# zyc-123/InstanceDiff

Hardware: AMD Instinct MI355X
Metric: denoising steps/sec (256x256 bs16) (higher is better)
Workload: dtype f32; 1 GPU; 256x256 1-ch synthetic, 1000-step reverse chain, batch 16 per GPU, 2 UNet fwd + reverse update per step; global_batch=16, parallelism=replicas x1 (no collective)

## Files before the change

### include/idiff.h

```cpp
#ifndef IDIFF_H
#define IDIFF_H

#include <stdint.h>

#ifdef __cplusplus
extern "C" {
#endif

#define IDIFF_OK 0
#define IDIFF_E_BADARG (-1)
#define IDIFF_E_UNSUPPORTED (-2)
#define IDIFF_E_HIP (-3)

typedef void* idiff_stream_t;

const char* idiff_last_error(void);
int idiff_version(void);
int64_t idiff_launch_count(void);
int idiff_device_info(int* num_cu, int* wave_size, char* arch_name, int arch_name_len);

#define IDIFF_CONV_NORMAL 0
#define IDIFF_CONV_UPSAMPLE2 1
#define IDIFF_CONV_UNSHUFFLE2 2

// ... 79 lines not shown
    const float* res;
    int64_t ldr;
    const float* gscale;
    float* out;
    int64_t ldo;
    const float* ln_g;
    const float* ln_b;
    float ln_eps;
    int32_t R, K, N, act_in, act_out;
} idiff_linear_group;
int idiff_linear_t_grouped_fwd(const idiff_linear_group* groups, int ngroups, idiff_stream_t stream);
int idiff_linear_t_ln_fwd(const float* x, int64_t ldx, const float* ln_g, const float* ln_b, float ln_eps, const float* wT,
                          int64_t ldw, const float* bias, const float* res, int64_t ldr, const float* gscale, float* out,
                          int64_t ldo, int R, int K, int N, int act_out, idiff_stream_t stream);
int idiff_linear_t_heads_fwd(const float* x, int64_t ldx, int64_t x_hs, const float* wT, int64_t ldw, int64_t w_hs,
                             const float* bias, int64_t b_hs, float* out, int64_t ldo, int64_t o_hs, int R, int K, int N,
                             int heads, idiff_stream_t stream);
int idiff_smm_memproj_fwd(const float* feat, int64_t feat_bstride, const float* ln1_g, const float* ln1_b,
                          const float* wpk, const float* bias, const float* ln2_g, const float* ln2_b, float* out, int B,
                          int C, int N, float eps, idiff_stream_t stream);
int idiff_smm_memproj_compact_fwd(const float* feat, int64_t feat_bstride, const float* ln1_g, const float* ln1_b,
                                  const float* gram, const float* hvec, float evar, float* out, int B, int C, int N, int Cm,
                                  float eps1, float eps2, idiff_stream_t stream);
int idiff_smm_memproj_compact_train_fwd(const float* feat, int64_t feat_bstride, const float* ln1_g, const float* ln1_b, const float* gram,
                                        const float* hvec, const float* evar_dev, float* out, int B, int C, int N, int Cm, float eps1,
                                        float eps2, idiff_stream_t stream);
int64_t idiff_smm_memproj_compact_bwd_ws_floats(int B, int C, int N);
int idiff_smm_memproj_compact_bwd(const float* feat, int64_t feat_bstride, const float* ln1_g, const float* ln1_b, const float* gram,
                                  const float* hvec, const float* evar_dev, const float* dm, float* dfeat, int64_t dfeat_bstride,
                                  float* dparams, float* ws, int B, int C, int N, int Cm, float eps1, float eps2, idiff_stream_t stream);
#define IDIFF_MEMPROJ_MAX_GROUPS 4
typedef struct idiff_memproj_group {
    const float* feat;
    int64_t feat_bstride;
    const float *ln1_g, *ln1_b, *gram, *hvec;
    float evar;
    float* out;
    int32_t C, N, Cm;
} idiff_memproj_group;
int idiff_smm_memproj_compact_grouped_fwd(const idiff_memproj_group* groups, int ngroups, int B, float eps1, float eps2,
                                          idiff_stream_t stream);
int idiff_layernorm_rows_fwd(const float* x, int64_t ldx, const float* gamma, const float* beta, float* out,
                             int64_t ldo, int R, int C, float eps, float* mean_rstd, idiff_stream_t stream);
int idiff_time_embed_fwd(const float* t, const float* freqs, int B, int dim, float* out, idiff_stream_t stream);
int idiff_time_mlp_fwd(const float* t, const float* freqs, const float* w0, const float* b0, const float* w2, const float* b2, float* out,
                       int B, int dim, int hid, int nout, idiff_stream_t stream);

int idiff_chan_layernorm_fwd(const float* x, int64_t x_bstride, const float* gamma, const float* beta, float* out,
                             int64_t out_bstride, int B, int C, int HW, float eps, float* mean_rstd,
                             idiff_stream_t stream);

int idiff_attn_self_fwd(const float* qkv, float* out, float* lse, int B, int C, int N, int heads, float scale,
                        idiff_stream_t stream);
int idiff_attn_self_bf16_fwd(const float* qkv, float* out, int B, int C, int N, int heads, float scale, idiff_stream_t stream);
int idiff_attn_self_f16_fwd(const float* qkv, float* out, int B, int C, int N, int heads, float scale, idiff_stream_t stream);
int idiff_attn_ctx_fwd(const float* q, const float* k, const float* v, float* out, int B, int C, int N, int M,
                       int heads, float scale, idiff_stream_t stream);
int idiff_attn_tokens_fwd(const float* q, const float* k, const float* v, float* out, int B, int Nq, int M, int C,
                          int heads, float scale, int64_t ldq, int64_t ldkv, idiff_stream_t stream);
int idiff_attn_tokens_bwd(const float* q, const float* k, const float* v, const float* d_o, float* dq, float* dk, float* dv, int B, int Nq,
                          int M, int C, int heads, float scale, int64_t ldq, int64_t ldkv, int64_t ldo, int64_t lddq, int64_t lddkv,
                          idiff_stream_t stream);
int idiff_attn_tokens_grouped_fwd(const float* const* q, const float* const* k, const float* const* v, float* const* out, int ngroups,
                                  int B, int Nq, int M, int C, int heads, float scale, int64_t ldq, int64_t ldkv, idiff_stream_t stream);
int idiff_attn_tokens_f16_fwd(const float* q, const float* k, const float* v, float* out, int B, int Nq, int M, int C, int heads, float scale,
                              int64_t ldq, int64_t ldkv, idiff_stream_t stream);
int64_t idiff_smm_xattn_kv_f16_ws_floats(int B, int N);
int idiff_smm_xattn_kv_f16_fwd(const float* q, const float* k, const float* v, float* out, float* ws, int B, int Nq, int heads, int C, int N,
                               float scale, idiff_stream_t stream);
int64_t idiff_smm_xattn_ws_floats(int B, int Nq, int heads, int Cm, int N);
int idiff_smm_xattn_fwd(const float* qf, const float* mem, float* o, float* ws, int B, int Nq, int heads, int Cm,
                        int N, float scale, idiff_stream_t stream);
#define IDIFF_XATTN_MAX_GROUPS 8
typedef struct idiff_xattn_group {
    const float* qf;
    const float* mem;
    float* o;
    float* ws;
    int32_t Cm, N;
} idiff_xattn_group;
int idiff_smm_xattn_grouped_fwd(const idiff_xattn_group* groups, int ngroups, int B, int Nq, int heads, float scale,
                                idiff_stream_t stream);
int idiff_smm_xattn_lse_fwd(const float* qf, const float* mem, float* o, float* lse, float* ws, int B, int rows, int N, float scale,
                            idiff_stream_t stream);
int idiff_smm_xattn_bwd(const float* qf, const float* mem, const float* o, const float* lse, const float* d_o, float* dqf, float* dmem,
                        int accumulate, float* ws, int B, int rows, int N, float scale, idiff_stream_t stream);
int idiff_smm_xattn_cm_lse_fwd(const float* qf, const float* mem, float* o, float* lse, float* ws, int B, int rows, int Cm, int N,
                               float scale, idiff_stream_t stream);
int idiff_smm_xattn_cm_bwd(const float* qf, const float* mem, const float* o, const float* lse, const float* d_o, float* dqf, float* dmem,
                           int accumulate, float* ws, int B, int rows, int Cm, int N, float scale, idiff_stream_t stream);
int idiff_scoremap_fwd(const float* feat, int64_t feat_bstride, const float* tv, float* out, const int32_t* idx,
                       float* sel, int B, int C, int HW, int K, idiff_stream_t stream);
#define IDIFF_SCOREMAP_MAX_GROUPS 4
typedef struct idiff_scoremap_group {
    const float* feat;
    int64_t feat_bstride;
    const float* tv;
    float* out;
    float* sel;
    int32_t C, HW;
} idiff_scoremap_group;
int idiff_scoremap_grouped_fwd(const idiff_scoremap_group* groups, int ngroups, const int32_t* idx, int B, int K, idiff_stream_t stream);
int idiff_conv3x3_select_fwd(const float* x, int64_t x_bstride, const float* w, const float* bias, const int32_t* idx, float* out,
                             int B, int C, int K, int H, int W, idiff_stream_t stream);
int64_t idiff_conv3x3_select_bwd_ws_floats(int B, int C, int H, int W);
int idiff_conv3x3_select_bwd(const float* x, int64_t x_bstride, const float* w, const int32_t* idx, const float* dpred, float* dx,
// ... 112 lines not shown
```

### instancediff_amd/_lib.py

```python
import ctypes as C
import os
import re

_HERE = os.path.dirname(os.path.abspath(__file__))
LIB_PATH = os.environ.get("IDIFF_LIB") or os.path.join(_HERE, "libidiff_hip.so")
HEADER_PATH = os.path.join(os.path.dirname(_HERE), "include", "idiff.h")

c_f32p = C.c_void_p
c_stream = C.c_void_p


class ConvDesc(C.Structure):
    _fields_ = [
        ("src0", C.c_void_p), ("src1", C.c_void_p),
        ("src0_bstride", C.c_int64), ("src1_bstride", C.c_int64),
        ("C0", C.c_int32), ("C1", C.c_int32),
        ("B", C.c_int32), ("Hin", C.c_int32), ("Win", C.c_int32),
        ("mode", C.c_int32), ("ks", C.c_int32), ("Cout", C.c_int32),
        ("wpk", C.c_void_p), ("bias", C.c_void_p),
        ("pro_a", C.c_void_p), ("pro_b", C.c_void_p),
        ("out", C.c_void_p), ("out_bstride", C.c_int64),
        ("res", C.c_void_p), ("res_bstride", C.c_int64),
        ("vec", C.c_void_p),
        ("aux", C.c_void_p), ("aux_bstride", C.c_int64), ("aux_a", C.c_void_p), ("aux_b", C.c_void_p),
# ... 15 lines not shown

class XattnGroup(C.Structure):
    _fields_ = [("qf", C.c_void_p), ("mem", C.c_void_p), ("o", C.c_void_p), ("ws", C.c_void_p), ("Cm", C.c_int32), ("N", C.c_int32)]


class MemprojGroup(C.Structure):
    _fields_ = [("feat", C.c_void_p), ("feat_bstride", C.c_int64), ("ln1_g", C.c_void_p), ("ln1_b", C.c_void_p), ("gram", C.c_void_p),
                ("hvec", C.c_void_p), ("evar", C.c_float), ("out", C.c_void_p), ("C", C.c_int32), ("N", C.c_int32), ("Cm", C.c_int32)]


class ScoremapGroup(C.Structure):
    _fields_ = [("feat", C.c_void_p), ("feat_bstride", C.c_int64), ("tv", C.c_void_p), ("out", C.c_void_p), ("sel", C.c_void_p),
                ("C", C.c_int32), ("HW", C.c_int32)]


LINEAR_MAX_GROUPS = 16
XATTN_MAX_GROUPS, MEMPROJ_MAX_GROUPS, SCOREMAP_MAX_GROUPS = 8, 4, 4
P, I, I64, F, U64 = C.c_void_p, C.c_int, C.c_int64, C.c_float, C.c_uint64

SIGNATURES = {
    "idiff_last_error": (C.c_char_p, []),
    "idiff_version": (I, []),
    "idiff_launch_count": (I64, []),
    "idiff_device_info": (I, [C.POINTER(I), C.POINTER(I), C.c_char_p, I]),
    "idiff_conv2d_num_tiles": (I, [I, I]),
    "idiff_conv2d_fwd": (I, [C.POINTER(ConvDesc), c_stream]),
    "idiff_conv2d_last_algo": (I, []),
    "idiff_conv2d_plan": (I, [C.POINTER(ConvDesc)]),
    "idiff_pack_conv_weight": (I, [P, P, I, I, I, c_stream]),
    "idiff_pack_conv_weight_T": (I, [P, P, I, I, I, c_stream]),
    "idiff_pack_conv_weight_wino": (I, [P, P, I, I, I, c_stream]),
    "idiff_pack_conv_weight_wino4": (I, [P, P, I, I, I, c_stream]),
    "idiff_conv1x1_x3_image_bytes": (C.c_longlong, [I, I]),
    "idiff_pack_conv1x1_x3": (I, [P, P, I, I, c_stream]),
    "idiff_gn_finalize": (I, [P, I, I, I, I, I, P, P, P, I64, F, P, P, P, c_stream]),
    "idiff_affine_silu_add": (I, [P, I64, P, P, P, I64, P, P, I64, I, I, I, c_stream]),
    "idiff_linear_fwd": (I, [P, I64, P, I64, P, P, I64, P, P, I64, I, I, I, I, I, c_stream]),
    "idiff_linear_t_fwd": (I, [P, I64, P, I64, P, P, I64, P, P, I64, I, I, I, I, I, c_stream]),
    "idiff_linear_t_ln_fwd": (I, [P, I64, P, P, F, P, I64, P, P, I64, P, P, I64, I, I, I, I, c_stream]),
    "idiff_linear_t_grouped_fwd": (I, [C.POINTER(LinearGroup), I, c_stream]),
    "idiff_attn_tokens_grouped_fwd": (I, [C.POINTER(P), C.POINTER(P), C.POINTER(P), C.POINTER(P), I, I, I, I, I, I, F, I64, I64, c_stream]),
    "idiff_linear_t_heads_fwd": (I, [P, I64, I64, P, I64, I64, P, I64, P, I64, I64, I, I, I, I, c_stream]),
    "idiff_smm_memproj_fwd": (I, [P, I64, P, P, P, P, P, P, P, I, I, I, F, c_stream]),
    "idiff_smm_memproj_compact_fwd": (I, [P, I64, P, P, P, P, F, P, I, I, I, I, F, F, c_stream]),
    "idiff_smm_memproj_compact_train_fwd": (I, [P, I64, P, P, P, P, P, P, I, I, I, I, F, F, c_stream]),
    "idiff_smm_memproj_compact_bwd_ws_floats": (I64, [I, I, I]),
    "idiff_smm_memproj_compact_bwd": (I, [P, I64, P, P, P, P, P, P, P, I64, P, P, I, I, I, I, F, F, c_stream]),
    "idiff_smm_memproj_compact_grouped_fwd": (I, [C.POINTER(MemprojGroup), I, I, F, F, c_stream]),
    "idiff_layernorm_rows_fwd": (I, [P, I64, P, P, P, I64, I, I, F, P, c_stream]),
    "idiff_time_embed_fwd": (I, [P, P, I, I, P, c_stream]),
    "idiff_time_mlp_fwd": (I, [P, P, P, P, P, P, P, I, I, I, I, c_stream]),
    "idiff_chan_layernorm_fwd": (I, [P, I64, P, P, P, I64, I, I, I, F, P, c_stream]),
    "idiff_attn_self_fwd": (I, [P, P, P, I, I, I, I, F, c_stream]),
    "idiff_attn_self_bf16_fwd": (I, [P, P, I, I, I, I, F, c_stream]),
    "idiff_attn_self_f16_fwd": (I, [P, P, I, I, I, I, F, c_stream]),
    "idiff_attn_ctx_fwd": (I, [P, P, P, P, I, I, I, I, I, F, c_stream]),
    "idiff_attn_tokens_fwd": (I, [P, P, P, P, I, I, I, I, I, F, I64, I64, c_stream]),
    "idiff_attn_tokens_bwd": (I, [P, P, P, P, P, P, P, I, I, I, I, I, F, I64, I64, I64, I64, I64, c_stream]),
    "idiff_smm_xattn_ws_floats": (I64, [I, I, I, I, I]),
    "idiff_attn_tokens_f16_fwd": (I, [P, P, P, P, I, I, I, I, I, F, I64, I64, c_stream]),
    "idiff_smm_xattn_kv_f16_ws_floats": (I64, [I, I]),
    "idiff_smm_xattn_kv_f16_fwd": (I, [P, P, P, P, P, I, I, I, I, I, F, c_stream]),
    "idiff_smm_xattn_fwd": (I, [P, P, P, P, I, I, I, I, I, F, c_stream]),
    "idiff_smm_xattn_grouped_fwd": (I, [C.POINTER(XattnGroup), I, I, I, I, F, c_stream]),
    "idiff_smm_xattn_lse_fwd": (I, [P, P, P, P, P, I, I, I, F, c_stream]),
    "idiff_smm_xattn_bwd": (I, [P, P, P, P, P, P, P, I, P, I, I, I, F, c_stream]),
    "idiff_smm_xattn_cm_lse_fwd": (I, [P, P, P, P, P, I, I, I, I, F, c_stream]),
    "idiff_smm_xattn_cm_bwd": (I, [P, P, P, P, P, P, P, I, P, I, I, I, I, F, c_stream]),
    "idiff_scoremap_fwd": (I, [P, I64, P, P, P, P, I, I, I, I, c_stream]),
    "idiff_scoremap_grouped_fwd": (I, [C.POINTER(ScoremapGroup), I, P, I, I, c_stream]),
    "idiff_gather_channel": (I, [P, P, P, I, I, I, c_stream]),
    "idiff_conv3x3_select_fwd": (I, [P, I64, P, P, P, P, I, I, I, I, I, c_stream]),
    "idiff_conv3x3_select_bwd_ws_floats": (I64, [I, I, I, I]),
    "idiff_conv3x3_select_bwd": (I, [P, I64, P, P, P, P, I64, P, P, P, I, I, I, I, I, c_stream]),
    "idiff_irsde_reverse_step": (I, [P, P, P, P, P, I64, F, F, F, F, F, I, U64, U64, c_stream]),
    "idiff_irsde_map": (I, [I, P, P, P, P, F, P, I, I64, P, C.POINTER(C.c_float), U64, U64, c_stream]),
    "idiff_drift_reverse_step": (I, [P, P, P, P, P, P, P, I64, F, F, F, U64, U64, c_stream]),
    "idiff_drift_reverse_step_dev": (I, [P, P, P, P, P, P, I64, P, I, P, U64, U64, U64, c_stream]),
    "idiff_step_state_advance": (I, [P, P, I, I, I, c_stream]),
    "idiff_randn": (I, [P, I64, U64, U64, c_stream]),
    "idiff_dropout": (I, [P, P, I64, F, U64, U64, c_stream]),
    "idiff_philox_raw": (I, [P, I64, U64, U64, c_stream]),
    "idiff_axpby": (I, [P, P, P, I64, F, F, c_stream]),
    "idiff_mix3_per_sample": (I, [P, P, P, P, P, P, P, I, I64, c_stream]),
    "idiff_conv2d_wgrad_ws_floats": (I64, [C.POINTER(ConvDesc)]),
    "idiff_conv2d_wgrad": (I, [C.POINTER(ConvDesc), P, I64, P, I, P, c_stream]),
    "idiff_conv2d_wgrad_last_algo": (I, []),
    "idiff_sumpool2x2": (I, [P, P, I64, I, I, c_stream]),
    "idiff_pixel_shuffle2": (I, [P, P, I, I, I, I, c_stream]),
    "idiff_plane_sum": (I, [P, I64, P, I, I, I, c_stream]),
    "idiff_batch_sum": (I, [P, P, I, I, I, c_stream]),
    "idiff_sum_n": (I, [C.POINTER(P), C.POINTER(I64), I, P, I64, I, I64, c_stream]),
    "idiff_gather_segments": (I, [P, I, I64, P, c_stream]),
    "idiff_gn_silu_bwd_ws_floats": (I64, [I, I, I]),
    "idiff_gn_silu_bwd": (I, [P, I64, P, I64, P, P, P, P, P, P, I64, P, I64, P, P, P, I64, P, I, I, I, I, I, P, P, c_stream]),
    "idiff_act_fwd": (I, [P, P, I64, I, c_stream]),
    "idiff_act_bwd": (I, [P, P, P, I64, I, c_stream]),
    "idiff_colsum": (I, [P, I64, P, I, I, I, c_stream]),
    "idiff_scale_cols": (I, [P, P, P, I, I, c_stream]),
    "idiff_colsum_prod": (I, [P, P, P, I, I, c_stream]),
    "idiff_layernorm_rows_bwd": (I, [P, I64, P, I64, P, P, P, I64, P, P, I, I, I, c_stream]),
    "idiff_chan_layernorm_bwd_ws_floats": (I64, [I, I, I]),
    "idiff_chan_layernorm_bwd": (I, [P, I64, P, I64, P, P, P, I64, P, P, P, I, I, I, I, c_stream]),
    "idiff_chan_normalize_fwd": (I, [P, I64, P, P, I, I, I, c_stream]),
    "idiff_chan_normalize_bwd": (I, [P, P, P, P, I64, I, I, I, c_stream]),
    "idiff_scatter_channel": (I, [P, P, P, I, I, I, c_stream]),
# ... 57 lines not shown
```

### instancediff_amd/csrc/attention.hip

```cpp
#include <math.h>
#include <type_traits>
#include <stdlib.h>

#include "common.h"

namespace {

#define KAPPA(r) (((r) & 3) + 8 * ((r) >> 2))

template <int DH>
__global__ __launch_bounds__(256) void attn_self_kernel(const float* __restrict__ qkv, float* __restrict__ out, float* __restrict__ lse, int C,
                                                        int N, int heads, float scale) {
    constexpr int MB = DH / 32;
    constexpr int KT = DH * 32;
    constexpr int VT = DH * 33;
    constexpr int BUF = KT + VT + 3;
    constexpr int NV4 = DH * 32 / 4 / 256;
    extern __shared__ __attribute__((aligned(16))) float smem[];

    const int tid = threadIdx.x, lane = tid & 63, wave = tid >> 6, half = lane >> 5, l31 = lane & 31;
    const int b = blockIdx.y / heads, h = blockIdx.y % heads;
    const int q0 = (blockIdx.x * 4 + wave) * 32;
    const float* qb = qkv + (long long)b * 3 * C * N + (long long)(h * DH) * N;
    const float* kb = qb + (long long)C * N;
    const float* vb = qb + (long long)2 * C * N;

    float qreg[DH / 2];
    const int qi = q0 + l31;
#pragma unroll
    for (int s = 0; s < DH / 2; ++s) qreg[s] = qi < N ? qb[(long long)(2 * s + half) * N + qi] : 0.f;

    floatx16 O[MB];
#pragma unroll
    for (int m = 0; m < MB; ++m)
#pragma unroll
        for (int r = 0; r < 16; ++r) O[m][r] = 0.f;
    float mrun = -INFINITY, lrun = 0.f;

    const int nkb = (N + 31) / 32;
    floatx4 rk[NV4], rv[NV4];
    auto load_tile = [&](int kbi) {
        const int key0 = kbi * 32;
#pragma unroll
        for (int i = 0; i < NV4; ++i) {
            const int f = tid + i * 256;
            const int d = f >> 3, j4 = (f & 7) * 4;
            floatx4 kz = {0.f, 0.f, 0.f, 0.f}, vz = {0.f, 0.f, 0.f, 0.f};
            if (key0 + j4 + 3 < N) {
                kz = *reinterpret_cast<const floatx4*>(kb + (long long)d * N + key0 + j4);
                vz = *reinterpret_cast<const floatx4*>(vb + (long long)d * N + key0 + j4);
            } else {
                for (int e = 0; e < 4; ++e)
                    if (key0 + j4 + e < N) {
                        kz[e] = kb[(long long)d * N + key0 + j4 + e];
                        vz[e] = vb[(long long)d * N + key0 + j4 + e];
                    }
            }
// ... 165 lines not shown
        for (int r = 0; r < 16; ++r) S[r] = 0.f;
#pragma unroll
        for (int s = 0; s < 4; ++s) {
            const bf16x8 ka = *reinterpret_cast<const bf16x8*>(kt + l31 * KROW + 16 * s + 8 * half);
            S = mfma_half<HT>(ka, qreg[s], S);
        }
        const int key0 = kbi * 32 + 4 * half;
        float mx = -INFINITY;
#pragma unroll
        for (int r = 0; r < 16; ++r) {
            const float sv = (key0 + KAPPA(r) < N) ? S[r] * scale : -INFINITY;
            S[r] = sv;
            mx = fmaxf(mx, sv);
        }
        mx = fmaxf(mx, __shfl_xor(mx, 32, 64));
        const float mnew = fmaxf(mrun, mx);
        const float alpha = __expf(mrun - mnew);
        float ps = 0.f;
        bf16x8 pb[2];
#pragma unroll
        for (int r = 0; r < 16; ++r) {
            const float p = __expf(S[r] - mnew);
            ps += p;
            pb[r >> 3][r & 7] = (HT)p;
        }
        lrun = lrun * alpha + ps;
        mrun = mnew;
        if (__any(alpha != 1.f)) {
#pragma unroll
            for (int m = 0; m < MB; ++m)
#pragma unroll
                for (int r = 0; r < 16; ++r) O[m][r] *= alpha;
        }
#pragma unroll
        for (int t = 0; t < 2; ++t)
#pragma unroll
            for (int m = 0; m < MB; ++m) {
                const HT* vr = vt + (m * 32 + l31) * VROW + 16 * t + 4 * half;
                const bf16x4 lo = *reinterpret_cast<const bf16x4*>(vr), hi = *reinterpret_cast<const bf16x4*>(vr + 8);
                const bf16x8 va = {lo[0], lo[1], lo[2], lo[3], hi[0], hi[1], hi[2], hi[3]};
                O[m] = mfma_half<HT>(va, pb[t], O[m]);
            }
        if (kbi + 1 < nkb) write_tile(buf ^ 1);
        __syncthreads();
    }
    const float l = lrun + __shfl_xor(lrun, 32, 64);
    const float inv = 1.0f / l;
    if (qi < N) {
        float* ob = out + (long long)b * C * N + (long long)(h * DH) * N + qi;
#pragma unroll
        for (int m = 0; m < MB; ++m)
#pragma unroll
            for (int r = 0; r < 16; ++r) ob[(long long)(m * 32 + KAPPA(r) + 4 * half) * N] = O[m][r] * inv;
    }
}

template <int DH>
__global__ __launch_bounds__(256) void attn_ctx_kernel(const float* __restrict__ q, const float* __restrict__ k, const float* __restrict__ v,
                                                       float* __restrict__ out, int C, int N, int M, float scale) {
    extern __shared__ float kv[];
    const int b = blockIdx.z, h = blockIdx.y;
    for (int i = threadIdx.x; i < M * DH; i += blockDim.x) {
        const int m = i / DH, d = i % DH;
        kv[i] = k[((long long)b * M + m) * C + h * DH + d];
        kv[M * DH + i] = v[((long long)b * M + m) * C + h * DH + d];
    }
    __syncthreads();
    const int p = blockIdx.x * blockDim.x + threadIdx.x;
    if (p >= N) return;
    const float* qp = q + ((long long)b * C + h * DH) * N + p;
    float qr[DH], o[DH];
#pragma unroll
    for (int d = 0; d < DH; ++d) {
        qr[d] = qp[(long long)d * N];
        o[d] = 0.f;
    }
    float mrun = -INFINITY, l = 0.f;
    for (int m = 0; m < M; ++m) {
        float s = 0.f;
#pragma unroll
        for (int d = 0; d < DH; ++d) s += qr[d] * kv[m * DH + d];
        s *= scale;
        const float mnew = fmaxf(mrun, s);
        const float alpha = __expf(mrun - mnew), pw = __expf(s - mnew);
        l = l * alpha + pw;
#pragma unroll
        for (int d = 0; d < DH; ++d) o[d] = o[d] * alpha + pw * kv[M * DH + m * DH + d];
        mrun = mnew;
    }
    const float inv = 1.0f / l;
    float* op = out + ((long long)b * C + h * DH) * N + p;
#pragma unroll
    for (int d = 0; d < DH; ++d) op[(long long)d * N] = o[d] * inv;
}

__global__ __launch_bounds__(64) void attn_tokens_kernel(const float* __restrict__ q, const float* __restrict__ k, const float* __restrict__ v,
                                                         float* __restrict__ out, int Nq, int M, int C, int heads, float scale, long long ldq,
                                                         long long ldkv) {
    const int dh = C / heads;
    const int n = blockIdx.x % Nq, h = (blockIdx.x / Nq) % heads, b = blockIdx.x / (Nq * heads);
    const int lane = threadIdx.x;
    const float* qp = q + ((long long)b * Nq + n) * ldq + h * dh;
    float s = -INFINITY;
    if (lane < M) {
        const float* kp = k + ((long long)b * M + lane) * ldkv + h * dh;
        float acc = 0.f;
// ... 597 lines not shown
                        if (cl < XCW) Dm[m][r] += dmemb[(long long)cl * N + key];
                    }
            }
#pragma unroll
            for (int m = 0; m < XCB; ++m)
#pragma unroll
                for (int r = 0; r < 16; ++r) {
                    const int cl = m * 32 + KAPPA(r) + 4 * half;
                    if (cl < XCW) dmemb[(long long)cl * N + key] = Dm[m][r];
                }
        }
        if (kbi + 1 < kb_end) write_tile();
        __syncthreads();
    }
    float* wp = ws + ((long long)b * nsplit + sp) * XCM * 32;
#pragma unroll
    for (int m = 0; m < XCB; ++m)
#pragma unroll
        for (int r = 0; r < 16; ++r) {
            const int cl = m * 32 + KAPPA(r) + 4 * half;
            if (cl < XCW) wp[(c0 + cl) * 32 + l31] = Oq[m][r];
        }
}

__global__ __launch_bounds__(256) void smm_xattn_bwd_combine_kernel(const float* __restrict__ ws, float* __restrict__ dqf, int rows, int nsplit, int XCM) {
    const int b = blockIdx.y;
    const int i = blockIdx.x * blockDim.x + threadIdx.x;
    const int c = i >> 5, row = i & 31;
    if (c >= XCM || row >= rows) return;
    const float* wb = ws + (long long)b * nsplit * XCM * 32;
    float acc = 0.f;
#pragma unroll 8
    for (int s = 0; s < nsplit; ++s) acc += wb[(long long)s * XCM * 32 + c * 32 + row];
    dqf[((long long)b * rows + row) * XCM + c] = acc;
}

inline void smm_split(int B, int N, int* nsplit, int* kps) {
    (void)B;
    static const int per = [] {
        const char* e = getenv("IDIFF_XATTN_SPLITS");
        return e && atoi(e) == 64 ? 64 : 32;
    }();
    const int nkb = (N + 31) / 32;
    int k = nkb / per;
    if (k < 2) k = 2;
    if (k > 2048 / per) k = 2048 / per;
    if (k > nkb) k = nkb;
    *kps = k;
    *nsplit = (nkb + k - 1) / k;
}

}

extern "C" int idiff_attn_self_fwd(const float* qkv, float* out, float* lse, int B, int C, int N, int heads, float scale, idiff_stream_t stream) {
    IDIFF_CHECK_ARG(qkv && out && B > 0 && C > 0 && N > 0 && heads > 0 && C % heads == 0, "attn_self: bad args");
    const int dh = C / heads;
    IDIFF_CHECK_ARG(dh == 64 || dh == 32, "attn_self: head dim must be 32 or 64 (got %d)", dh);
    IDIFF_CHECK_ARG(N % 4 == 0, "attn_self: N must be a multiple of 4");
    dim3 grid((N + 127) / 128, B * heads);
    hipStream_t st = (hipStream_t)stream;
    if (dh == 64) {
        const size_t lds = 2 * (64 * 32 + 64 * 33 + 3) * sizeof(float);
        hipLaunchKernelGGL(attn_self_kernel<64>, grid, dim3(256), lds, st, qkv, out, lse, C, N, heads, scale);
    } else {
        const size_t lds = 2 * (32 * 32 + 32 * 33 + 3) * sizeof(float);
        hipLaunchKernelGGL(attn_self_kernel<32>, grid, dim3(256), lds, st, qkv, out, lse, C, N, heads, scale);
    }
    IDIFF_CHECK_LAUNCH("attn_self_fwd");
    return IDIFF_OK;
}

extern "C" int idiff_attn_self_bf16_fwd(const float* qkv, float* out, int B, int C, int N, int heads, float scale, idiff_stream_t stream) {
    IDIFF_CHECK_ARG(qkv && out && B > 0 && C > 0 && N > 0 && heads > 0 && C % heads == 0, "attn_self_bf16: bad args");
    IDIFF_CHECK_ARG(C / heads == 64, "attn_self_bf16: head dim must be 64 (got %d)", C / heads);
    IDIFF_CHECK_ARG(N % 4 == 0 && (reinterpret_cast<uintptr_t>(qkv) & 15) == 0, "attn_self_bf16: N %% 4 and 16-byte alignment required");
    dim3 grid((N + 127) / 128, B * heads);
    const size_t lds = (size_t)2 * (32 * (64 + 8) + 64 * (32 + 4)) * sizeof(uint16_t);
    hipLaunchKernelGGL(attn_self_half_kernel<__bf16>, grid, dim3(256), lds, (hipStream_t)stream, qkv, out, C, N, heads, scale);
    IDIFF_CHECK_LAUNCH("attn_self_bf16_fwd");
    return IDIFF_OK;
}

extern "C" int idiff_attn_self_f16_fwd(const float* qkv, float* out, int B, int C, int N, int heads, float scale, idiff_stream_t stream) {
    IDIFF_CHECK_ARG(qkv && out && B > 0 && C > 0 && N > 0 && heads > 0 && C % heads == 0, "attn_self_f16: bad args");
    IDIFF_CHECK_ARG(C / heads == 64, "attn_self_f16: head dim must be 64 (got %d)", C / heads);
    IDIFF_CHECK_ARG(N % 4 == 0 && (reinterpret_cast<uintptr_t>(qkv) & 15) == 0, "attn_self_f16: N %% 4 and 16-byte alignment required");
    dim3 grid((N + 127) / 128, B * heads);
    const size_t lds = (size_t)2 * (32 * (64 + 8) + 64 * (32 + 4)) * sizeof(uint16_t);
    hipLaunchKernelGGL(attn_self_half_kernel<_Float16>, grid, dim3(256), lds, (hipStream_t)stream, qkv, out, C, N, heads, scale);
    IDIFF_CHECK_LAUNCH("attn_self_f16_fwd");
    return IDIFF_OK;
}

extern "C" int idiff_attn_ctx_fwd(const float* q, const float* k, const float* v, float* out, int B, int C, int N, int M, int heads, float scale,
                                  idiff_stream_t stream) {
    IDIFF_CHECK_ARG(q && k && v && out && B > 0 && C > 0 && N > 0 && heads > 0 && C % heads == 0, "attn_ctx: bad args");
    IDIFF_CHECK_ARG(M >= 1 && M <= 32, "attn_ctx: M must be in 1..32 (got %d)", M);
    const int dh = C / heads;
    dim3 grid((N + 255) / 256, heads, B);
    const size_t lds = (size_t)2 * M * dh * sizeof(float);
    hipStream_t st = (hipStream_t)stream;
    if (dh == 16)
        hipLaunchKernelGGL(attn_ctx_kernel<16>, grid, dim3(256), lds, st, q, k, v, out, C, N, M, scale);
    else if (dh == 32)
        hipLaunchKernelGGL(attn_ctx_kernel<32>, grid, dim3(256), lds, st, q, k, v, out, C, N, M, scale);
    else if (dh == 64)
        hipLaunchKernelGGL(attn_ctx_kernel<64>, grid, dim3(256), lds, st, q, k, v, out, C, N, M, scale);
    else
        IDIFF_FAIL(IDIFF_E_UNSUPPORTED, "attn_ctx: head dim must be 16, 32 or 64 (got %d)", dh);
    IDIFF_CHECK_LAUNCH("attn_ctx_fwd");
    return IDIFF_OK;
}

extern "C" int idiff_attn_tokens_fwd(const float* q, const float* k, const float* v, float* out, int B, int Nq, int M, int C, int heads,
                                     float scale, int64_t ldq, int64_t ldkv, idiff_stream_t stream) {
    IDIFF_CHECK_ARG(q && k && v && out && B > 0 && Nq > 0 && C > 0 && heads > 0 && C % heads == 0, "attn_tokens: bad args");
    IDIFF_CHECK_ARG(M >= 1 && M <= 64, "attn_tokens: M must be in 1..64 (got %d)", M);
    IDIFF_CHECK_ARG(ldq >= C && ldkv >= C, "attn_tokens: row strides must be >= C");
    hipLaunchKernelGGL(attn_tokens_kernel, dim3(B * heads * Nq), dim3(64), 0, (hipStream_t)stream, q, k, v, out, Nq, M, C, heads, scale,
                       (long long)ldq, (long long)ldkv);
    IDIFF_CHECK_LAUNCH("attn_tokens_fwd");
    return IDIFF_OK;
// ... 164 lines not shown
```

### instancediff_amd/csrc/conv1x1_x3.hip

```cpp
#include <stdlib.h>

#include <type_traits>

#include "conv_args.h"

using idiff_detail::ConvArgs;

namespace {

typedef unsigned uintx4 __attribute__((ext_vector_type(4)));
typedef __bf16 bf16x8 __attribute__((ext_vector_type(8)));

constexpr int BM = 64, CKB = 32, NT = 256;
constexpr int B_ISTR = 1088;
constexpr int B_KGSTR = 4 * B_ISTR;
constexpr int B_PLSTR = 4 * B_KGSTR;
constexpr int B_BYTES = 3 * B_PLSTR;
constexpr int A_PLSTR = 4 * 64 * 16;
constexpr int A_BYTES = 3 * A_PLSTR;
constexpr int OLD = 256 + 4;
static_assert(32 * OLD * 4 <= B_BYTES, "epilogue tile must fit in the B planes");

__host__ __device__ constexpr unsigned hi16(unsigned u) { return u & 0xffff0000u; }

__device__ __forceinline__ unsigned pack_hi(unsigned odd, unsigned even) { return __builtin_amdgcn_perm(odd, even, 0x07060302u); }

__device__ __forceinline__ void split3(const float (&x)[8], uintx4& p1, uintx4& p2, uintx4& p3) {
    unsigned u1[8], u2[8], u3[8];
#pragma unroll
    for (int c = 0; c < 8; ++c) {
        u1[c] = __builtin_bit_cast(unsigned, x[c]);
        const float r1 = x[c] - __builtin_bit_cast(float, hi16(u1[c]));
        u2[c] = __builtin_bit_cast(unsigned, r1);
        const float r2 = r1 - __builtin_bit_cast(float, hi16(u2[c]));
        u3[c] = __builtin_bit_cast(unsigned, r2);
    }
    p1 = uintx4{pack_hi(u1[1], u1[0]), pack_hi(u1[3], u1[2]), pack_hi(u1[5], u1[4]), pack_hi(u1[7], u1[6])};
    p2 = uintx4{pack_hi(u2[1], u2[0]), pack_hi(u2[3], u2[2]), pack_hi(u2[5], u2[4]), pack_hi(u2[7], u2[6])};
    p3 = uintx4{pack_hi(u3[1], u3[0]), pack_hi(u3[3], u3[2]), pack_hi(u3[5], u3[4]), pack_hi(u3[7], u3[6])};
}

template <typename T>
__device__ __forceinline__ T* scalar_ptr(const T* p) {
    const unsigned long long v = reinterpret_cast<unsigned long long>(p);
    const unsigned lo = __builtin_amdgcn_readfirstlane((unsigned)v), hi = __builtin_amdgcn_readfirstlane((unsigned)(v >> 32));
    return reinterpret_cast<T*>(((unsigned long long)hi << 32) | lo);
}

__device__ __forceinline__ floatx4 mma(const uintx4& a, const uintx4& b, const floatx4& c) {
    return __builtin_amdgcn_mfma_f32_16x16x32_bf16(__builtin_bit_cast(bf16x8, a), __builtin_bit_cast(bf16x8, b), c, 0, 0, 0);
}

template <bool UNSH>
__global__ __launch_bounds__(NT) __attribute__((amdgpu_waves_per_eu(2, 2))) void conv1x1_x3_kernel(const ConvArgs a, const unsigned short* __restrict__ wx3) {
    extern __shared__ __attribute__((aligned(16))) unsigned char smem_raw[];
    unsigned char* const Bs = smem_raw;
    unsigned char* const As = smem_raw + B_BYTES;
    float* const econst = reinterpret_cast<float*>(smem_raw + B_BYTES + A_BYTES);

    const int tid = threadIdx.x;
    const int lane = tid & 63;
    const int wave = __builtin_amdgcn_readfirstlane(tid >> 6);
    const int n16 = lane & 15, kgl = lane >> 4;

    const unsigned logical = xcd_remap(blockIdx.x, a.total_wg);
    const int cob = logical % a.ncob;
    const int tile = (logical / a.ncob) % a.ntiles;
    const int b = logical / (a.ncob * a.ntiles);
    const int co0 = cob * BM;
    const long long HW = (long long)a.Hout * a.Wout;
    const long long pix0 = (long long)tile * 256;

    {
        const int which = tid >> 6, co = co0 + (tid & 63);
        float v = 0.f;
        if (which == 0 && a.bias) v = a.bias[co];
        if (which == 1 && a.vec) v = a.vec[(long long)b * a.Cout + co];
        if (which == 2 && a.aux) v = a.aux_a[(long long)b * a.Cout + co];
        if (which == 3 && a.aux) v = a.aux_b[(long long)b * a.Cout + co];
        econst[tid] = v;
    }

    const int q = lane, kg = wave;
    const int nchunks = (a.Cin + CKB - 1) / CKB;
    floatx4 xrA[8], xrB[8];
    uintx4 ar[3];
    constexpr int RSRC_FLAGS = 0x00020000;
    const float* const s0 = a.src0 + (long long)b * a.bs0 + (UNSH ? 0 : pix0);
    const float* const s1 = a.src1 ? a.src1 + (long long)b * a.bs1 + pix0 : s0;
    const long long HWin = (long long)a.Hin * a.Win;
    const int chstride_b = (int)((UNSH ? HWin : HW) * 4);
    int xoff = q * 16;
    if (UNSH) {
// ... 231 lines not shown
```

Measured before the change: 43.84 steps/s.

## Run f32 self-attention on bf16 MFMA with three-way split emulation

```diff
diff --git a/include/idiff.h b/include/idiff.h
--- a/include/idiff.h
+++ b/include/idiff.h
@@ -155,6 +155,10 @@
 
 int idiff_attn_self_fwd(const float* qkv, float* out, float* lse, int B, int C, int N, int heads, float scale,
                         idiff_stream_t stream);
+int idiff_attn_self_f32_fwd(const float* qkv, float* out, float* lse, int B, int C, int N, int heads, float scale,
+                            idiff_stream_t stream);
+int idiff_attn_self_x3_fwd(const float* qkv, float* out, float* lse, int B, int C, int N, int heads, float scale,
+                           idiff_stream_t stream);
 int idiff_attn_self_bf16_fwd(const float* qkv, float* out, int B, int C, int N, int heads, float scale, idiff_stream_t stream);
 int idiff_attn_self_f16_fwd(const float* qkv, float* out, int B, int C, int N, int heads, float scale, idiff_stream_t stream);
 int idiff_attn_ctx_fwd(const float* q, const float* k, const float* v, float* out, int B, int C, int N, int M,
diff --git a/instancediff_amd/_lib.py b/instancediff_amd/_lib.py
--- a/instancediff_amd/_lib.py
+++ b/instancediff_amd/_lib.py
@@ -91,6 +91,8 @@
     "idiff_time_mlp_fwd": (I, [P, P, P, P, P, P, P, I, I, I, I, c_stream]),
     "idiff_chan_layernorm_fwd": (I, [P, I64, P, P, P, I64, I, I, I, F, P, c_stream]),
     "idiff_attn_self_fwd": (I, [P, P, P, I, I, I, I, F, c_stream]),
+    "idiff_attn_self_f32_fwd": (I, [P, P, P, I, I, I, I, F, c_stream]),
+    "idiff_attn_self_x3_fwd": (I, [P, P, P, I, I, I, I, F, c_stream]),
     "idiff_attn_self_bf16_fwd": (I, [P, P, I, I, I, I, F, c_stream]),
     "idiff_attn_self_f16_fwd": (I, [P, P, I, I, I, I, F, c_stream]),
     "idiff_attn_ctx_fwd": (I, [P, P, P, P, I, I, I, I, I, F, c_stream]),
diff --git a/instancediff_amd/csrc/attention.hip b/instancediff_amd/csrc/attention.hip
--- a/instancediff_amd/csrc/attention.hip
+++ b/instancediff_amd/csrc/attention.hip
@@ -3,6 +3,7 @@
 #include <stdlib.h>
 
 #include "common.h"
+#include "split_x3.h"
 
 namespace {
 
@@ -274,6 +275,173 @@
         for (int m = 0; m < MB; ++m)
 #pragma unroll
             for (int r = 0; r < 16; ++r) ob[(long long)(m * 32 + KAPPA(r) + 4 * half) * N] = O[m][r] * inv;
+    }
+}
+
+__device__ __forceinline__ floatx16 mma_x3(const uintx4& a, const uintx4& b, const floatx16& c) {
+    typedef __bf16 bf16x8v __attribute__((ext_vector_type(8)));
+    return __builtin_amdgcn_mfma_f32_32x32x16_bf16(__builtin_bit_cast(bf16x8v, a), __builtin_bit_cast(bf16x8v, b), c, 0, 0, 0);
+}
+__device__ __forceinline__ floatx16 mma6(const uintx4 (&a)[3], const uintx4 (&b)[3], floatx16 c) {
+    c = mma_x3(a[2], b[0], c);
+    c = mma_x3(a[1], b[1], c);
+    c = mma_x3(a[0], b[2], c);
+    c = mma_x3(a[1], b[0], c);
+    c = mma_x3(a[0], b[1], c);
+    return mma_x3(a[0], b[0], c);
+}
+
+constexpr int AX3_KROW = 64 + 8;
+constexpr int AX3_VROW = 32 + 4;
+constexpr int AX3_KT = 32 * AX3_KROW;
+constexpr int AX3_VT = 64 * AX3_VROW;
+constexpr int AX3_BUF = 3 * (AX3_KT + AX3_VT);
+
+__global__ __launch_bounds__(256) __attribute__((amdgpu_waves_per_eu(2, 2))) void attn_self_x3_kernel(const float* __restrict__ qkv, float* __restrict__ out, float* __restrict__ lse, int C,
+                                                          int N, int heads, float scale) {
+    constexpr int DH = 64, MB = 2;
+    extern __shared__ __attribute__((aligned(16))) unsigned short x3sm[];
+    const int tid = threadIdx.x, lane = tid & 63, wave = tid >> 6, half = lane >> 5, l31 = lane & 31;
+    const int b = blockIdx.y / heads, h = blockIdx.y % heads;
+    const int q0 = (blockIdx.x * 4 + wave) * 32;
+    const float* qb = qkv + (long long)b * 3 * C * N + (long long)(h * DH) * N;
+    const float* kb = qb + (long long)C * N;
+    const float* vb = qb + (long long)2 * C * N;
+    const int qi = q0 + l31;
+    uintx4 qx[4][3];
+#pragma unroll
+    for (int s = 0; s < 4; ++s) {
+        float qv[8];
+#pragma unroll
+        for (int e = 0; e < 8; ++e) qv[e] = qi < N ? qb[(long long)(16 * s + 8 * half + e) * N + qi] : 0.f;
+        split3(qv, qx[s][0], qx[s][1], qx[s][2]);
+    }
+    floatx16 O[MB];
+#pragma unroll
+    for (int m = 0; m < MB; ++m)
+#pragma unroll
+        for (int r = 0; r < 16; ++r) O[m][r] = 0.f;
+    float mrun = -INFINITY, lrun = 0.f;
+    const int nkb = (N + 31) / 32;
+    floatx4 rk[2], rv[2];
+    auto load_tile = [&](int kbi) {
+        const int key0 = kbi * 32;
+#pragma unroll
+        for (int i = 0; i < 2; ++i) {
+            const int f = tid + i * 256;
+            const int d = f >> 3, j4 = (f & 7) * 4;
+            floatx4 kz = {0.f, 0.f, 0.f, 0.f}, vz = {0.f, 0.f, 0.f, 0.f};
+            if (key0 + j4 + 3 < N) {
+                kz = *reinterpret_cast<const floatx4*>(kb + (long long)d * N + key0 + j4);
+                vz = *reinterpret_cast<const floatx4*>(vb + (long long)d * N + key0 + j4);
+            } else {
+                for (int e = 0; e < 4; ++e)
+                    if (key0 + j4 + e < N) kz[e] = kb[(long long)d * N + key0 + j4 + e], vz[e] = vb[(long long)d * N + key0 + j4 + e];
+            }
+            rk[i] = kz, rv[i] = vz;
+        }
+    };
+    auto write_tile = [&](int buf) {
+        unsigned short* kt = x3sm + buf * AX3_BUF;
+        unsigned short* vt = kt + 3 * AX3_KT;
+#pragma unroll
+        for (int i = 0; i < 2; ++i) {
+            const int f = tid + i * 256;
+            const int d = f >> 3, j4 = (f & 7) * 4;
+            unsigned uk[3][4], uv[3][4];
+#pragma unroll
+            for (int e = 0; e < 4; ++e) {
+                split3_words(rk[i][e], uk[0][e], uk[1][e], uk[2][e]);
+                split3_words(rv[i][e], uv[0][e], uv[1][e], uv[2][e]);
+            }
+#pragma unroll
+            for (int p = 0; p < 3; ++p) {
+#pragma unroll
+                for (int e = 0; e < 4; ++e) kt[p * AX3_KT + (j4 + e) * AX3_KROW + d] = (unsigned short)(uk[p][e] >> 16);
+                *reinterpret_cast<uintx2*>(vt + p * AX3_VT + d * AX3_VROW + j4) = uintx2{pack_hi(uv[p][1], uv[p][0]), pack_hi(uv[p][3], uv[p][2])};
+            }
+        }
+    };
+    load_tile(0);
+    write_tile(0);
+    __syncthreads();
+    for (int kbi = 0; kbi < nkb; ++kbi) {
+        const int buf = kbi & 1;
+        if (kbi + 1 < nkb) load_tile(kbi + 1);
+        const unsigned short* kt = x3sm + buf * AX3_BUF;
+        const unsigned short* vt = kt + 3 * AX3_KT;
+        floatx16 S;
+#pragma unroll
+        for (int r = 0; r < 16; ++r) S[r] = 0.f;
+#pragma unroll
+        for (int s = 0; s < 4; ++s) {
+            uintx4 ka[3];
+#pragma unroll
+            for (int p = 0; p < 3; ++p) ka[p] = *reinterpret_cast<const uintx4*>(kt + p * AX3_KT + l31 * AX3_KROW + 16 * s + 8 * half);
+            S = mma6(ka, qx[s], S);
+        }
+        float mx = -INFINITY;
+#pragma unroll
+        for (int r = 0; r < 16; ++r) {
+            S[r] *= scale;
+            mx = fmaxf(mx, S[r]);
+        }
+        if (kbi * 32 + 32 > N) {
+            const int key0 = kbi * 32 + 4 * half;
+            mx = -INFINITY;
+#pragma unroll
+            for (int r = 0; r < 16; ++r) {
+                S[r] = (key0 + KAPPA(r) < N) ? S[r] : -INFINITY;
+                mx = fmaxf(mx, S[r]);
+            }
+        }
+        mx = fmaxf(mx, __shfl_xor(mx, 32, 64));
+        const float mnew = fmaxf(mrun, mx);
+        const float alpha = __expf(mrun - mnew);
+        float ps = 0.f;
+        float pv[2][8];
+#pragma unroll
+        for (int r = 0; r < 16; ++r) {
+            const float p = __expf(S[r] - mnew);
+            ps += p;
+            pv[r >> 3][r & 7] = p;
+        }
+        uintx4 px[2][3];
+#pragma unroll
+        for (int t = 0; t < 2; ++t) split3(pv[t], px[t][0], px[t][1], px[t][2]);
+        lrun = lrun * alpha + ps;
+        mrun = mnew;
+        if (__any(alpha != 1.f)) {
+#pragma unroll
+            for (int m = 0; m < MB; ++m)
+#pragma unroll
+                for (int r = 0; r < 16; ++r) O[m][r] *= alpha;
+        }
+#pragma unroll
+        for (int t = 0; t < 2; ++t)
+#pragma unroll
+            for (int m = 0; m < MB; ++m) {
+                uintx4 va[3];
+#pragma unroll
+                for (int p = 0; p < 3; ++p) {
+                    const unsigned short* vr = vt + p * AX3_VT + (m * 32 + l31) * AX3_VROW + 16 * t + 4 * half;
+                    const uintx2 lo = *reinterpret_cast<const uintx2*>(vr), hi = *reinterpret_cast<const uintx2*>(vr + 8);
+                    va[p] = uintx4{lo.x, lo.y, hi.x, hi.y};
+                }
+                O[m] = mma6(va, px[t], O[m]);
+            }
+        if (kbi + 1 < nkb) write_tile(buf ^ 1);
+        __syncthreads();
+    }
+    const float l = lrun + __shfl_xor(lrun, 32, 64);
+    const float inv = 1.0f / l;
+    if (qi < N) {
+        float* ob = out + (long long)b * C * N + (long long)(h * DH) * N + qi;
+#pragma unroll
+        for (int m = 0; m < MB; ++m)
+#pragma unroll
+            for (int r = 0; r < 16; ++r) ob[(long long)(m * 32 + KAPPA(r) + 4 * half) * N] = O[m][r] * inv;
+        if (lse && half == 0) lse[((long long)b * heads + h) * N + qi] = mrun + logf(l);
     }
 }
 
@@ -977,22 +1145,46 @@
 
 }
 
-extern "C" int idiff_attn_self_fwd(const float* qkv, float* out, float* lse, int B, int C, int N, int heads, float scale, idiff_stream_t stream) {
-    IDIFF_CHECK_ARG(qkv && out && B > 0 && C > 0 && N > 0 && heads > 0 && C % heads == 0, "attn_self: bad args");
+static int attn_self_fwd_impl(const float* qkv, float* out, float* lse, int B, int C, int N, int heads, float scale, idiff_stream_t stream,
+                              int form, const char* name) {
+    IDIFF_CHECK_ARG(qkv && out && B > 0 && C > 0 && N > 0 && heads > 0 && C % heads == 0, "%s: bad args", name);
     const int dh = C / heads;
-    IDIFF_CHECK_ARG(dh == 64 || dh == 32, "attn_self: head dim must be 32 or 64 (got %d)", dh);
-    IDIFF_CHECK_ARG(N % 4 == 0, "attn_self: N must be a multiple of 4");
+    IDIFF_CHECK_ARG(dh == 64 || dh == 32, "%s: head dim must be 32 or 64 (got %d)", name, dh);
+    IDIFF_CHECK_ARG(N % 4 == 0, "%s: N must be a multiple of 4", name);
+    IDIFF_CHECK_ARG(form != 2 || dh == 64, "%s: the x3 form needs head dim 64 (got %d)", name, dh);
+    static const bool x3_on = [] {
+        const char* e = getenv("IDIFF_X3_ATTN");
+        return !e || atoi(e) != 0;
+    }();
     dim3 grid((N + 127) / 128, B * heads);
     hipStream_t st = (hipStream_t)stream;
-    if (dh == 64) {
+    if (dh == 64 && (form == 2 || (form == 0 && x3_on))) {
+        const size_t lds = (size_t)2 * AX3_BUF * sizeof(uint16_t);
+        static idiff_dyn_lds_cache lds_cache;
+        const hipError_t e = idiff_ensure_dyn_lds(lds_cache, reinterpret_cast<const void*>(attn_self_x3_kernel), lds);
+        if (e != hipSuccess) IDIFF_FAIL(IDIFF_E_HIP, "%s: hipFuncSetAttribute: %s", name, hipGetErrorString(e));
+        hipLaunchKernelGGL(attn_self_x3_kernel, grid, dim3(256), lds, st, qkv, out, lse, C, N, heads, scale);
+    } else if (dh == 64) {
         const size_t lds = 2 * (64 * 32 + 64 * 33 + 3) * sizeof(float);
         hipLaunchKernelGGL(attn_self_kernel<64>, grid, dim3(256), lds, st, qkv, out, lse, C, N, heads, scale);
     } else {
         const size_t lds = 2 * (32 * 32 + 32 * 33 + 3) * sizeof(float);
         hipLaunchKernelGGL(attn_self_kernel<32>, grid, dim3(256), lds, st, qkv, out, lse, C, N, heads, scale);
     }
-    IDIFF_CHECK_LAUNCH("attn_self_fwd");
+    IDIFF_CHECK_LAUNCH(name);
     return IDIFF_OK;
+}
+
+extern "C" int idiff_attn_self_fwd(const float* qkv, float* out, float* lse, int B, int C, int N, int heads, float scale, idiff_stream_t stream) {
+    return attn_self_fwd_impl(qkv, out, lse, B, C, N, heads, scale, stream, 0, "attn_self_fwd");
+}
+
+extern "C" int idiff_attn_self_f32_fwd(const float* qkv, float* out, float* lse, int B, int C, int N, int heads, float scale, idiff_stream_t stream) {
+    return attn_self_fwd_impl(qkv, out, lse, B, C, N, heads, scale, stream, 1, "attn_self_f32_fwd");
+}
+
+extern "C" int idiff_attn_self_x3_fwd(const float* qkv, float* out, float* lse, int B, int C, int N, int heads, float scale, idiff_stream_t stream) {
+    return attn_self_fwd_impl(qkv, out, lse, B, C, N, heads, scale, stream, 2, "attn_self_x3_fwd");
 }
 
 extern "C" int idiff_attn_self_bf16_fwd(const float* qkv, float* out, int B, int C, int N, int heads, float scale, idiff_stream_t stream) {
diff --git a/instancediff_amd/csrc/conv1x1_x3.hip b/instancediff_amd/csrc/conv1x1_x3.hip
--- a/instancediff_amd/csrc/conv1x1_x3.hip
+++ b/instancediff_amd/csrc/conv1x1_x3.hip
@@ -3,12 +3,12 @@
 #include <type_traits>
 
 #include "conv_args.h"
+#include "split_x3.h"
 
 using idiff_detail::ConvArgs;
 
 namespace {
 
-typedef unsigned uintx4 __attribute__((ext_vector_type(4)));
 typedef __bf16 bf16x8 __attribute__((ext_vector_type(8)));
 
 constexpr int BM = 64, CKB = 32, NT = 256;
@@ -20,25 +20,6 @@
 constexpr int A_BYTES = 3 * A_PLSTR;
 constexpr int OLD = 256 + 4;
 static_assert(32 * OLD * 4 <= B_BYTES, "epilogue tile must fit in the B planes");
-
-__host__ __device__ constexpr unsigned hi16(unsigned u) { return u & 0xffff0000u; }
-
-__device__ __forceinline__ unsigned pack_hi(unsigned odd, unsigned even) { return __builtin_amdgcn_perm(odd, even, 0x07060302u); }
-
-__device__ __forceinline__ void split3(const float (&x)[8], uintx4& p1, uintx4& p2, uintx4& p3) {
-    unsigned u1[8], u2[8], u3[8];
-#pragma unroll
-    for (int c = 0; c < 8; ++c) {
-        u1[c] = __builtin_bit_cast(unsigned, x[c]);
-        const float r1 = x[c] - __builtin_bit_cast(float, hi16(u1[c]));
-        u2[c] = __builtin_bit_cast(unsigned, r1);
-        const float r2 = r1 - __builtin_bit_cast(float, hi16(u2[c]));
-        u3[c] = __builtin_bit_cast(unsigned, r2);
-    }
-    p1 = uintx4{pack_hi(u1[1], u1[0]), pack_hi(u1[3], u1[2]), pack_hi(u1[5], u1[4]), pack_hi(u1[7], u1[6])};
-    p2 = uintx4{pack_hi(u2[1], u2[0]), pack_hi(u2[3], u2[2]), pack_hi(u2[5], u2[4]), pack_hi(u2[7], u2[6])};
-    p3 = uintx4{pack_hi(u3[1], u3[0]), pack_hi(u3[3], u3[2]), pack_hi(u3[5], u3[4]), pack_hi(u3[7], u3[6])};
-}
 
 template <typename T>
 __device__ __forceinline__ T* scalar_ptr(const T* p) {
diff --git a/instancediff_amd/csrc/split_x3.h b/instancediff_amd/csrc/split_x3.h
--- /dev/null
+++ b/instancediff_amd/csrc/split_x3.h
@@ -0,0 +1,26 @@
+#pragma once
+#include <hip/hip_runtime.h>
+
+typedef unsigned uintx4 __attribute__((ext_vector_type(4)));
+typedef unsigned uintx2 __attribute__((ext_vector_type(2)));
+
+__host__ __device__ constexpr unsigned hi16(unsigned u) { return u & 0xffff0000u; }
+
+__device__ __forceinline__ unsigned pack_hi(unsigned odd, unsigned even) { return __builtin_amdgcn_perm(odd, even, 0x07060302u); }
+
+__device__ __forceinline__ void split3_words(float x, unsigned& u1, unsigned& u2, unsigned& u3) {
+    u1 = __builtin_bit_cast(unsigned, x);
+    const float r1 = x - __builtin_bit_cast(float, hi16(u1));
+    u2 = __builtin_bit_cast(unsigned, r1);
+    const float r2 = r1 - __builtin_bit_cast(float, hi16(u2));
+    u3 = __builtin_bit_cast(unsigned, r2);
+}
+
+__device__ __forceinline__ void split3(const float (&x)[8], uintx4& p1, uintx4& p2, uintx4& p3) {
+    unsigned u1[8], u2[8], u3[8];
+#pragma unroll
+    for (int c = 0; c < 8; ++c) split3_words(x[c], u1[c], u2[c], u3[c]);
+    p1 = uintx4{pack_hi(u1[1], u1[0]), pack_hi(u1[3], u1[2]), pack_hi(u1[5], u1[4]), pack_hi(u1[7], u1[6])};
+    p2 = uintx4{pack_hi(u2[1], u2[0]), pack_hi(u2[3], u2[2]), pack_hi(u2[5], u2[4]), pack_hi(u2[7], u2[6])};
+    p3 = uintx4{pack_hi(u3[1], u3[0]), pack_hi(u3[3], u3[2]), pack_hi(u3[5], u3[4]), pack_hi(u3[7], u3[6])};
+}
```

Measured after the change: 44.07 steps/s, median of 6. Within noise of the previous version (+0.5%).
